# DOGECOIN87/firedancer

Hardware: AMD Instinct MI355X
Metric: verified ed25519 sigs/sec (node) (higher is better)
Workload: dtype u32; 1 GPU; cfg2: 1000000 single-sig txns/GPU, msg U[180,220] B, 90% valid / 10% corrupted, device-resident batch, full verify + per-txn combine per step; parallelism=dp1 (independent per-GPU batches), queues=2

## Files before the change

firedancer_amd/csrc/fdgpu_internal.h:

```cpp
#pragma once

#include <hip/hip_runtime_api.h>
#include <stddef.h>
#include <stdint.h>

#include "../../include/fd_ed25519_gpu.h"
#include "../../include/fd_poh_gpu.h"

typedef struct {
  uint32_t msg_off;
  uint32_t msg_sz;
  uint32_t sig_off;
  uint32_t pub_off;
} fdgpu_sig_desc_t;

typedef struct {
  uint32_t sig0;
  uint32_t sig_cnt;
} fdgpu_txn_desc_t;

#define FDGPU_ARENA_SLACK   160u
#define FDGPU_ATAB_ENTRIES  9u
#ifndef FDGPU_ATAB_WORDS
#define FDGPU_ATAB_WORDS    40u
#endif
#define FDGPU_PTAB_WORDS    32u
#ifndef FDGPU_VERIFY_WAVES
#define FDGPU_VERIFY_WAVES  2
#endif
#ifndef FDGPU_PHASE_STAMPS
#define FDGPU_PHASE_STAMPS  0
#endif
#define FDGPU_BCOMB_BITS    16u
#define FDGPU_BCOMB_NDIG    ((254u + FDGPU_BCOMB_BITS - 1u) / FDGPU_BCOMB_BITS)
#define FDGPU_BCOMB_ENTRIES ((1u << (FDGPU_BCOMB_BITS - 1u)) + 1u)
#define FDGPU_BCOMB_STRIDE  32u
#define FDGPU_BCOMB_CHUNK   64u
#define HS_MAX_WIN          40u
#define FDGPU_TAB_STORED    (FDGPU_ATAB_ENTRIES - 1u)
#define FDGPU_WS_RTAB       FDGPU_TAB_STORED
#define FDGPU_WS_ENTRIES    (2u * FDGPU_TAB_STORED + 2u)
#define FDGPU_WS_LANE_WORDS (FDGPU_WS_ENTRIES * FDGPU_ATAB_WORDS)
#define FDGPU_WS_TAB_WORDS  (2u * FDGPU_TAB_STORED * FDGPU_PTAB_WORDS)
#define FDGPU_WS_AUX_WORDS  (FDGPU_WS_LANE_WORDS - FDGPU_WS_TAB_WORDS)
#define FDGPU_AUX_PARK      0u
#define FDGPU_AUX_SB        FDGPU_ATAB_WORDS
#define FDGPU_BLOCK         256u
#define FDGPU_FLAG_REF_MAP  1u
#define FDGPU_FLAG_KFULL    2u
#define FDGPU_FLAG_KCACHE   4u
#define FDGPU_FLAG_KPAIR    8u
#define FDGPU_FLAG_KSPREAD  16u
#define FDGPU_STAGE_WAVE_WORDS (FDGPU_PTAB_WORDS / 4u * 256u)
#define FDGPU_STAGE_LDS        (FDGPU_BLOCK / 64u * 2u * FDGPU_STAGE_WAVE_WORDS * 4u)
#define FDGPU_STAGE_LDS_PAIR   (FDGPU_BLOCK / 64u * FDGPU_STAGE_WAVE_WORDS * 4u)
#define FDGPU_CU_LDS           (160u * 1024u)
#define FDGPU_SPREAD_LDS       (FDGPU_CU_LDS / 2u - FDGPU_STAGE_LDS + 1024u)
#define FDGPU_SPREAD_LDS_PAIR  (FDGPU_CU_LDS / 2u - FDGPU_STAGE_LDS_PAIR + 1024u)
#ifdef __cplusplus
static_assert(2u * (FDGPU_STAGE_LDS + FDGPU_SPREAD_LDS) > FDGPU_CU_LDS &&
              2u * (FDGPU_STAGE_LDS_PAIR + FDGPU_SPREAD_LDS_PAIR) > FDGPU_CU_LDS &&
              FDGPU_STAGE_LDS + FDGPU_SPREAD_LDS <= FDGPU_CU_LDS && FDGPU_STAGE_LDS_PAIR + FDGPU_SPREAD_LDS_PAIR <= FDGPU_CU_LDS,
              "a spread launch's LDS admits one block per CU, and no more");
#endif
#define FDGPU_FULL_BLOCKS   16u
#define FDGPU_AUX_BLOCKS    64u
#define FDGPU_IO_BLOCKS     16u
#define FDGPU_NBLK_GROUPS   32u
#define FDGPU_POH_CHUNK     64u

#ifdef __cplusplus
extern "C" {
#endif


size_t     fdgpu_btab_bytes(void);
hipError_t fdgpu_btab_build(uint32_t *d_btab, hipStream_t stream);

hipError_t fdgpu_launch_verify_sigs(const uint8_t *d_arena, const fdgpu_sig_desc_t *d_sigs, uint32_t n_sig,
// ... 116 lines not shown
```

firedancer_amd/csrc/fdgpu_verify.hip:

```cpp
#include <hip/hip_runtime.h>

#include "fdgpu_atab.h"
#include "fdgpu_bcomb.h"
#include "fdgpu_ge.h"
#include "fdgpu_hram.h"
#include "fdgpu_internal.h"
#include "fdgpu_lattice.h"
#include "fdgpu_sc.h"
#include "fdgpu_sha512.h"
#include "fdgpu_stamps.h"

using namespace fdgpu;

namespace {


FDG_DEV uint32_t *tab_a(uint32_t *wsl) { return wsl - FDGPU_PTAB_WORDS; }
FDG_DEV const uint32_t *tab_a(const uint32_t *wsl) { return wsl - FDGPU_PTAB_WORDS; }
FDG_DEV uint32_t *tab_r(uint32_t *wsl) { return wsl + (FDGPU_WS_RTAB - 1u) * FDGPU_PTAB_WORDS; }

FDG_DEV void sb_store(uint32_t *aux, const ge_cached &c) {
  uint4 *p = (uint4 *)(aux + FDGPU_AUX_SB);
  uint32_t w[40];
#pragma unroll
  for (int i = 0; i < 10; i++) { w[i] = c.YpX.v[i]; w[10 + i] = c.YmX.v[i]; w[20 + i] = c.Z2.v[i]; w[30 + i] = c.T2d.v[i]; }
#pragma unroll
  for (int q = 0; q < 10; q++) p[q] = make_uint4(w[4 * q], w[4 * q + 1], w[4 * q + 2], w[4 * q + 3]);
}
FDG_DEV void sb_load(uint32_t (&q)[40], const uint32_t *aux) {
  const uint4 *ent = (const uint4 *)(aux + FDGPU_AUX_SB);
#pragma unroll
  for (int i = 0; i < 10; i++) {
    const uint4 v = ent[i];
    q[4 * i] = v.x; q[4 * i + 1] = v.y; q[4 * i + 2] = v.z; q[4 * i + 3] = v.w;
  }
}
FDG_DEV int sext4(uint32_t x) { return ((int)(x << 28)) >> 28; }

#define KD_WORDS 8

FDG_DEV void shl4(uint32_t (&w)[8]) {
#pragma unroll
  for (int i = 7; i > 0; i--) w[i] = (w[i] << 4) | (w[i - 1] >> 28);
  w[0] <<= 4;
}

FDG_DEV void dsm_k(ge_p2 &acc2, uint32_t (&kd)[KD_WORDS], const uint32_t *aux, const uint32_t *ta) {
  ge_p3 acc3;
  ge_p1p1 t;
  uint32_t q[40];
  {
    const int e = sext4(kd[7] >> 28);
    shl4(kd);
    atab_load(q, ta, e);
    ge_cached_regs_to_p2(acc2, q, e < 0);
  }
#pragma unroll 1
  for (int j = 62; j >= 0; j--) {
    const int e = sext4(kd[7] >> 28);
    shl4(kd);
    atab_load(q, ta, e);
#pragma unroll 1
    for (int r = 0; r < 4; r++) {
      ge_dbl(t, acc2);
      ge_p1p1_to_p2(acc2, t);
    }
    acc3.X = acc2.X; acc3.Y = acc2.Y; acc3.Z = acc2.Z; fe_mul(acc3.T, t.X, t.Y);
    ge_add_cached_regs(t, acc3, q, e < 0);
    if (j == 0) break;
    ge_p1p1_to_p2(acc2, t);
  }
  ge_p1p1_to_p3(acc3, t);
  uint32_t qs[40];
  sb_load(qs, aux);
  ge_add_cached_regs(t, acc3, qs, false);
  ge_p1p1_to_p2(acc2, t);
}

FDG_DEV void comb_sb(ge_p3 &acc, const uint32_t (&S)[8], const uint32_t *__restrict__ btab, uint32_t lo = 0,
                     uint32_t hi = BC_NDIG) {
  constexpr int NW = COMB_WORDS(BC_W, BC_NDIG), SLOT = COMB_SLOT(BC_W);
  uint32_t dg[NW];
  sc_recode_comb<(int)BC_W, (int)BC_NDIG>(dg, S);
  auto next_digit = [&dg]() {
    const int d = SLOT == 16 ? (int)(int16_t)(dg[0] & 0xffffu) : (int)dg[0];
#pragma unroll
    for (int i = 0; i < NW - 1; i++) dg[i] = SLOT == 16 ? (dg[i] >> 16) | (dg[i + 1] << 16) : dg[i + 1];
    dg[NW - 1] = SLOT == 16 ? dg[NW - 1] >> 16 : 0u;
    return d;
  };
  auto load_entry = [btab](uint32_t (&q)[32], uint32_t ti, int d) {
    const uint4 *ent = (const uint4 *)(btab + ((size_t)ti * BC_ENT + (uint32_t)(d < 0 ? -d : d)) * FDGPU_BCOMB_STRIDE);
#pragma unroll
    for (int i = 0; i < 8; i++) {
      const uint4 v = ent[i];
      q[4 * i] = v.x; q[4 * i + 1] = v.y; q[4 * i + 2] = v.z; q[4 * i + 3] = v.w;
    }
  };
  uint32_t qa[32], qb[32];
#pragma unroll 1
  for (uint32_t i = 0; i < lo; i++) (void)next_digit();
  int d = next_digit();
  load_entry(qa, lo, d);
  {
    const int dn = next_digit();
    load_entry(qb, lo + 1, dn);
    ge_niels_regs_to_p3(acc, qa, d < 0);
#pragma unroll
    for (int w = 0; w < 32; w++) qa[w] = qb[w];
    d = dn;
  }
  ge_p1p1 t;
#pragma unroll 1
  for (uint32_t i = lo + 1; i < hi; i++) {
    const int dn = next_digit();
    if (i + 1 < hi) load_entry(qb, i + 1, dn);
    ge_add_niels_regs(t, acc, qa, d < 0);
    ge_p1p1_to_p3(acc, t);
#pragma unroll
    for (int w = 0; w < 32; w++) qa[w] = qb[w];
    d = dn;
  }
}

FDG_DEV void atab_build(uint32_t *wsl, const ge_p3 &An) {
  ge_cached c;
  ge_p3_to_cached(c, An); atab_store(wsl, 1, c);
  ge_p1p1 t; ge_p2 a2; ge_p3 P;
  ge_p3_to_p2(a2, An); ge_dbl(t, a2); ge_p1p1_to_p3(P, t);
  ge_p3_to_cached(c, P); atab_store(wsl, 2, c);
  const uint32_t *ent1 = wsl + 1u * FDGPU_PTAB_WORDS;
  auto ld1 = [ent1](int cc, int w) { return atab_limb(ent1, cc, w); };
#pragma unroll 1
  for (uint32_t e = 3; e < FDGPU_ATAB_ENTRIES; e++) {
    if (e & 1u) {
      ge_add_cached_ld(t, P, ld1, false);
    } else {
      uint32_t q[40];
      atab_load(q, wsl, (int)(e >> 1));
      ge_cached_regs_to_p2(a2, q, false);
      ge_dbl(t, a2);
    }
    ge_p1p1_to_p3(P, t);
    ge_p3_to_cached(c, P); atab_store(wsl, e, c);
  }
}

FDG_DEV uint32_t *lane_ws(uint32_t *ws, uint32_t i) {
  return ws + (size_t)i * FDGPU_WS_TAB_WORDS;
}
FDG_DEV uint32_t *lane_aux(uint32_t *queue, uint32_t i) {
  return queue - ((size_t)i + 1u) * FDGPU_WS_AUX_WORDS;
}
FDG_DEV const uint32_t *lane_aux(const uint32_t *queue, uint32_t i) {
  return queue - ((size_t)i + 1u) * FDGPU_WS_AUX_WORDS;
}

FDG_DEV uint32_t out_idx(const uint32_t *__restrict__ perm, uint32_t i) { return perm ? perm[i] : i; }


#define HPARK_KD 0
#define HPARK_CODE 30
static_assert(HPARK_KD + KD_WORDS <= HPARK_CODE && HPARK_CODE < (int)FDGPU_AUX_SB - (int)FDGPU_AUX_PARK &&
              FDGPU_AUX_SB + FDGPU_ATAB_WORDS <= FDGPU_WS_AUX_WORDS && FDGPU_AUX_SB % 4u == 0 && FDGPU_WS_AUX_WORDS % 4u == 0,
              "aux layout");

FDG_DEV void recode16_160(uint32_t (&out)[5], uint32_t &nd, const uint32_t (&m)[5]) {
  uint32_t carry = 0;
  nd = 0;
#pragma unroll
  for (int w = 0; w < 5; w++) {
    uint32_t o = 0;
#pragma unroll
    for (int n = 0; n < 8; n++) {
      uint32_t e = ((m[w] >> (4 * n)) & 15u) + carry;
      carry = e >= 8u;
      e = (e - (carry << 4)) & 15u;
      o |= e << (4 * n);
      nd = e ? (uint32_t)(8 * w + n + 1) : nd;
    }
    out[w] = o;
  }
  nd = carry ? 41u : nd;
}

FDG_DEV void shl4_5(uint32_t (&w)[5]) {
#pragma unroll
  for (int i = 4; i > 0; i--) w[i] = (w[i] << 4) | (w[i - 1] >> 28);
  w[0] <<= 4;
}

FDG_DEV void hs_wscalar(uint32_t (&w)[8], const uint32_t (&v)[5], bool v_neg, const uint32_t (&S)[8]) {
  uint32_t x[16];
#pragma unroll
  for (int i = 0; i < 16; i++) x[i] = 0;
#pragma unroll
  for (int i = 0; i < 5; i++) {
// ... 61 lines not shown
    ge_p1p1_to_p3(acc3, t);
    unstage_entry_signed(q, st_r, (dv < 0) != v_neg);
    ge_add_cached_regs_swapped(t, acc3, q, (dv < 0) != v_neg);
  }
}


FDG_DEV uint32_t decode_neg_table(uint32_t *tab, const uint32_t (&enc)[8], bool ref_map) {
  ge_p3 P, Pn;
  const bool ok = ge_decode(P, enc, ref_map);
  const bool small = ge_is_small_order_affine(P);
  ge_p3_neg(Pn, P);
  atab_build(tab, Pn);
  return (ok ? 1u : 0u) | (small ? 2u : 0u);
}

FDG_DEV void hs_split_masked(hs_split_t &hs, const uint32_t (&k)[8], bool need) {
  uint32_t ke[8];
#pragma unroll
  for (int j = 0; j < 8; j++) ke[j] = need ? k[j] : 0u;
  hs_split(hs, ke);
}

FDG_DEV uint32_t hs_digits(uint32_t (&ud)[5], uint32_t (&vd)[5], const hs_split_t &hs) {
  uint32_t ndu = 0, ndv = 0;
  recode16_160(ud, ndu, hs.u);
  recode16_160(vd, ndv, hs.v);
  return max(max(ndu, ndv), 1u);
}

FDG_DEV void comb_scalar(uint32_t (&w)[8], const hs_split_t &hs, const uint32_t (&S)[8], bool half) {
  hs_wscalar(w, hs.v, hs.v_neg, S);
#pragma unroll
  for (int j = 0; j < 8; j++) w[j] = half ? w[j] : S[j];
}

FDG_DEV void park_full(uint32_t *park, const uint32_t (&k)[8]) {
  uint32_t kd[KD_WORDS];
  sc_recode16(kd, k);
#pragma unroll
  for (int j = 0; j < KD_WORDS; j++) park[HPARK_KD + j] = kd[j];
  park[HPARK_CODE] = 0u;
}

FDG_DEV void queue_full_lanes(uint32_t *queue, uint32_t *queue_cnt, bool q_full, uint32_t i) {
  const uint64_t m = __ballot(q_full);
  if (m) {
    const int lane = (int)(threadIdx.x & 63u);
    const int leader = __ffsll((long long)m) - 1;
    uint32_t base = 0;
    if (lane == leader) base = atomicAdd(queue_cnt, (uint32_t)__popcll(m));
    base = (uint32_t)__shfl((int)base, leader, 64);
    if (q_full) queue[base + (uint32_t)__popcll(m & ((1ull << lane) - 1ull))] = i;
  }
}

template <bool KC, bool PH = false>
FDG_DEV void verify_hs_body(const uint8_t *__restrict__ arena, const fdgpu_sig_desc_t *__restrict__ sigs, uint32_t n_sig_arg,
                            const uint32_t *__restrict__ n_sig_dev, const uint32_t *__restrict__ btab,
                            uint32_t *__restrict__ ws, const uint32_t *__restrict__ perm, int8_t *__restrict__ codes,
                            uint32_t *__restrict__ queue, uint32_t *__restrict__ queue_cnt, uint32_t flags,
                            const uint32_t *__restrict__ key_of, const uint32_t *__restrict__ kverd, uint32_t bx) {
  const uint32_t n_sig = n_sig_dev ? *n_sig_dev : n_sig_arg;
  if (bx * blockDim.x >= n_sig) return;
  const uint32_t i = bx * blockDim.x + threadIdx.x;
  const bool active = i < n_sig;
  const bool ref_map = (flags & FDGPU_FLAG_REF_MAP) != 0;
  const fdgpu_sig_desc_t d = sigs[active ? i : n_sig - 1];
  uint32_t nb = sha512_hram_blocks(d.msg_sz);
#pragma unroll
  for (int off = 32; off > 0; off >>= 1) nb = max(nb, (uint32_t)__shfl_xor((int)nb, off));
  uint32_t *wsl = lane_ws(ws, i);
  uint32_t *aux = lane_aux(queue, i);
  const uint32_t *ta = tab_a(wsl);
  FDGPU_STAMP(0);
  uint32_t Renc[8], Aenc[8];
  load32(Renc, arena + d.sig_off);
  load32(Aenc, arena + d.pub_off);
  uint32_t k[8];
  {
    uint64_t h[8];
    if (PH) {
#pragma unroll
      for (int j = 0; j < 8; j++) h[j] = ((const uint64_t *)(arena + d.msg_off))[j];
    } else {
      sha512_hram(h, Renc, Aenc, arena + d.msg_off, d.msg_sz, nb);
    }
    FDGPU_STAMP(1);
    uint32_t kx[16];
#pragma unroll
    for (int j = 0; j < 8; j++) { kx[2 * j] = bswap32((uint32_t)(h[j] >> 32)); kx[2 * j + 1] = bswap32((uint32_t)h[j]); }
    sc_reduce512(k, kx);
  }
  uint32_t S[8];
  load32(S, arena + d.sig_off + 32);
  int code = sc_lt_L(S) ? 0 : -1;
#pragma unroll
  for (int j = 0; j < 8; j++) S[j] = code ? 0u : S[j];
  FDGPU_STAMP(2);
  {
    ge_p3 P, Pn;
    bool a_ok, a_small;
    if (KC) {
      const uint32_t di = active ? i : n_sig - 1u, r = key_of[di], vd = kverd[r];
      a_ok = (vd & 1u) != 0;
      a_small = (vd & 2u) != 0;
      ta = tab_a(lane_ws(ws, r));
    } else {
      a_ok = ge_decode(P, Aenc, ref_map);
      a_small = ge_is_small_order_affine(P);
      ge_p3_neg(Pn, P);
      atab_build(tab_a(wsl), Pn);
    }
    FDGPU_STAMP(3);
    const bool r_ok = ge_decode(P, Renc, ref_map);
    const bool r_small = ge_is_small_order_affine(P);
    ge_p3_neg(Pn, P);
    atab_build(tab_r(wsl), Pn);
    if (code == 0 && !a_ok) code = ref_map ? -2 : -1;
    if (code == 0 && !r_ok) code = -1;
    if (code == 0 && a_small) code = -2;
    if (code == 0 && r_small) code = -1;
  }
  FDGPU_STAMP(4);
  const bool need = active && code == 0;
  hs_split_t hs;
  hs_split_masked(hs, k, need);
  uint32_t ud[5], vd[5];
  const uint32_t nd_lane = hs_digits(ud, vd, hs);
  const bool full = need && (!hs.ok || nd_lane > HS_MAX_WIN || (flags & FDGPU_FLAG_KFULL));
  const bool half = need && !full;
  FDGPU_STAMP(5);
  {
    uint32_t w[8];
    comb_scalar(w, hs, S, half);
    ge_p3 WB;
    comb_sb(WB, w, btab);
    ge_cached c; ge_p3_to_cached(c, WB);
    sb_store(aux, c);
  }
  if (full) park_full(aux + FDGPU_AUX_PARK, k);
  FDGPU_STAMP(6);
  bool eq = false;
  if (__any(half)) {
    const uint32_t nwin = wave_max_u32(half ? nd_lane : 1u);
#pragma unroll 1
    for (uint32_t s = nwin; s < 40; s++) { shl4_5(ud); shl4_5(vd); }
    ge_p1p1 t;
    hs_chain(t, ud, vd, hs.u_neg, hs.v_neg, nwin, wsl, ta);
    uint32_t q[40];
    sb_load(q, aux);
    fe ypx, ymx, z2, xw, yw, l1, l2;
#pragma unroll
    for (int j = 0; j < 10; j++) { ypx.v[j] = q[j]; ymx.v[j] = q[10 + j]; z2.v[j] = q[20 + j]; }
    fe_sub(xw, ypx, ymx);
    fe_add(yw, ypx, ymx);
    fe_mul(l1, t.X, z2);
    fe_mul(l2, t.Z, xw);
    fe_add(l1, l1, l2);
    const bool ex = fe_iszero(l1);
    fe_mul(l1, t.Y, z2);
    fe_mul(l2, t.T, yw);
    fe_sub(l1, l1, l2);
    eq = ex && fe_iszero(l1);
  }
  FDGPU_STAMP(7);
  if (active && !full) codes[out_idx(perm, i)] = (int8_t)(code ? code : (eq ? 0 : -3));
  queue_full_lanes(queue, queue_cnt, full, i);
}

template <bool KC, bool PH = false>
__global__ void __launch_bounds__(FDGPU_BLOCK, FDGPU_VERIFY_WAVES)
fdgpu_verify_hs_kernel(const uint8_t *__restrict__ arena, const fdgpu_sig_desc_t *__restrict__ sigs, uint32_t n_sig_arg,
                       const uint32_t *__restrict__ n_sig_dev, const uint32_t *__restrict__ btab,
                       uint32_t *__restrict__ ws, const uint32_t *__restrict__ perm, int8_t *__restrict__ codes,
                       uint32_t *__restrict__ queue, uint32_t *__restrict__ queue_cnt, uint32_t flags,
                       const uint32_t *__restrict__ key_of, const uint32_t *__restrict__ kverd) {
  verify_hs_body<KC, PH>(arena, sigs, n_sig_arg, n_sig_dev, btab, ws, perm, codes, queue, queue_cnt, flags, key_of,
                         kverd, blockIdx.x);
}

__global__ void __launch_bounds__(64) fdgpu_sha512_stream_kernel(const uint8_t *__restrict__ mbuf, uint64_t m0,
                                                                 uint64_t mlen, uint64_t msg_sz, uint64_t blk0,
                                                                 uint32_t nblk, const uint8_t *__restrict__ ra,
                                                                 uint64_t *__restrict__ state, uint32_t n) {
  const uint32_t i = threadIdx.x;
  if (i >= n) return;
  const uint64_t H0[8] = {0x6a09e667f3bcc908ULL, 0xbb67ae8584caa73bULL, 0x3c6ef372fe94f82bULL,
                          0xa54ff53a5f1d36f1ULL, 0x510e527fade682d1ULL, 0x9b05688c2b3e6c1fULL,
                          0x1f83d9abfb41bd6bULL, 0x5be0cd19137e2179ULL};
  uint64_t h[8];
  for (int j = 0; j < 8; j++) h[j] = blk0 ? state[8 * i + j] : H0[j];
  const uint64_t total = (64u + msg_sz + 16u) / 128u + 1u, bitlen = (64u + msg_sz) * 8u;
  for (uint64_t b = blk0; b < blk0 + nblk; b++) {
    uint64_t w[16];
    for (int t = 0; t < 16; t++) {
      uint64_t v = 0;
// ... 47 lines not shown
    stage_entry(st, tab, d);
#pragma unroll 1
    for (int r = 0; r < 4; r++) {
      ge_dbl(t, acc2);
      ge_p1p1_to_p2(acc2, t);
    }
    acc3.X = acc2.X; acc3.Y = acc2.Y; acc3.Z = acc2.Z; fe_mul(acc3.T, t.X, t.Y);
    asm volatile("s_waitcnt vmcnt(0)" ::: "memory");
    unstage_entry_signed(q, st, (d < 0) != neg);
    ge_add_cached_regs_swapped(t, acc3, q, (d < 0) != neg);
  }
}

FDG_DEV void fe_xchg_pair(fe &r, const fe &a) {
#pragma unroll
  for (int j = 0; j < 10; j++) r.v[j] = (uint32_t)__shfl_xor((int)a.v[j], 1);
}

template <bool PH = false>
__global__ void __launch_bounds__(FDGPU_BLOCK, FDGPU_VERIFY_WAVES)
fdgpu_verify_pair_kernel(const uint8_t *__restrict__ arena, const fdgpu_sig_desc_t *__restrict__ sigs, uint32_t n_sig_arg,
                         const uint32_t *__restrict__ n_sig_dev, const uint32_t *__restrict__ btab,
                         uint32_t *__restrict__ ws, const uint32_t *__restrict__ perm, int8_t *__restrict__ codes,
                         uint32_t *__restrict__ queue, uint32_t *__restrict__ queue_cnt, uint32_t flags) {
  const uint32_t n_sig = n_sig_dev ? *n_sig_dev : n_sig_arg;
  if (blockIdx.x * (blockDim.x / 2u) >= n_sig) return;
  const uint32_t g = blockIdx.x * blockDim.x + threadIdx.x, i = g >> 1;
  const bool rl = (g & 1u) != 0;
  const bool active = i < n_sig;
  const bool ref_map = (flags & FDGPU_FLAG_REF_MAP) != 0;
  const fdgpu_sig_desc_t d = sigs[active ? i : n_sig - 1];
  const uint32_t nb = wave_max_u32(sha512_hram_blocks(d.msg_sz));
  uint32_t *wsl = lane_ws(ws, i);
  uint32_t *aux = lane_aux(queue, i);
  uint32_t *tab = rl ? tab_r(wsl) : tab_a(wsl);
  uint32_t Renc[8], Aenc[8];
  load32(Renc, arena + d.sig_off);
  load32(Aenc, arena + d.pub_off);
  uint32_t k[8];
  if (PH) {
    uint32_t kx[16];
#pragma unroll
    for (int j = 0; j < 8; j++) {
      const uint64_t h = ((const uint64_t *)(arena + d.msg_off))[j];
      kx[2 * j] = bswap32((uint32_t)(h >> 32)); kx[2 * j + 1] = bswap32((uint32_t)h);
    }
    sc_reduce512(k, kx);
  } else {
    hram_k(k, Renc, Aenc, arena, d, nb);
  }
  uint32_t S[8];
  load32(S, arena + d.sig_off + 32);
  int code = sc_lt_L(S) ? 0 : -1;
#pragma unroll
  for (int j = 0; j < 8; j++) S[j] = code ? 0u : S[j];
  {
    uint32_t enc[8];
#pragma unroll
    for (int j = 0; j < 8; j++) enc[j] = rl ? Renc[j] : Aenc[j];
    const uint32_t mine = decode_neg_table(tab, enc, ref_map);
    const uint32_t other = (uint32_t)__shfl_xor((int)mine, 1);
    const uint32_t av = rl ? other : mine, rv = rl ? mine : other;
    if (code == 0 && !(av & 1u)) code = ref_map ? -2 : -1;
    if (code == 0 && !(rv & 1u)) code = -1;
    if (code == 0 && (av & 2u)) code = -2;
    if (code == 0 && (rv & 2u)) code = -1;
  }
  const bool need = active && code == 0;
  hs_split_t hs;
  hs_split_masked(hs, k, need);
  uint32_t ud[5], vd[5];
  const uint32_t nd_lane = hs_digits(ud, vd, hs);
  const bool full = need && (!hs.ok || nd_lane > HS_MAX_WIN || (flags & FDGPU_FLAG_KFULL));
  const bool half = need && !full;
  {
    uint32_t w[8];
    comb_scalar(w, hs, S, half);
    ge_p3 WB, WBo;
    comb_sb(WB, w, btab, rl ? BC_NDIG / 2u : 0u, rl ? BC_NDIG : BC_NDIG / 2u);
    fe_xchg_pair(WBo.X, WB.X);
    fe_xchg_pair(WBo.Y, WB.Y);
    fe_xchg_pair(WBo.Z, WB.Z);
    fe_xchg_pair(WBo.T, WB.T);
    ge_cached c; ge_p3_to_cached(c, WBo);
    ge_p1p1 tw; ge_add_cached(tw, WB, c, false);
    ge_p1p1_to_p3(WB, tw);
    ge_p3_to_cached(c, WB);
    if (!rl) sb_store(aux, c);
  }
  if (full && !rl) park_full(aux + FDGPU_AUX_PARK, k);
  bool eq = false;
  if (__any(half)) {
    const uint32_t nwin = wave_max_u32(half ? nd_lane : 1u);
    uint32_t dd[5];
#pragma unroll
    for (int j = 0; j < 5; j++) dd[j] = rl ? vd[j] : ud[j];
#pragma unroll 1
    for (uint32_t s2 = nwin; s2 < 40; s2++) shl4_5(dd);
    ge_p1p1 t;
    hs_chain1(t, dd, rl ? hs.v_neg : hs.u_neg, nwin, tab);
    ge_p3 mine, other;
    ge_p1p1_to_p3(mine, t);
    fe_xchg_pair(other.X, mine.X);
    fe_xchg_pair(other.Y, mine.Y);
    fe_xchg_pair(other.Z, mine.Z);
    fe_xchg_pair(other.T, mine.T);
    ge_cached oc;
    ge_p3_to_cached(oc, other);
    ge_add_cached(t, mine, oc, false);
    uint32_t q[40];
    sb_load(q, aux);
    fe ypx, ymx, z2, xw, yw, l1, l2;
#pragma unroll
    for (int j = 0; j < 10; j++) { ypx.v[j] = q[j]; ymx.v[j] = q[10 + j]; z2.v[j] = q[20 + j]; }
    fe_sub(xw, ypx, ymx);
    fe_add(yw, ypx, ymx);
    fe_mul(l1, t.X, z2);
    fe_mul(l2, t.Z, xw);
    fe_add(l1, l1, l2);
    const bool ex = fe_iszero(l1);
    fe_mul(l1, t.Y, z2);
    fe_mul(l2, t.T, yw);
    fe_sub(l1, l1, l2);
    eq = ex && fe_iszero(l1);
  }
  if (active && !full && !rl) codes[out_idx(perm, i)] = (int8_t)(code ? code : (eq ? 0 : -3));
  queue_full_lanes(queue, queue_cnt, full && !rl, i);
}

#define KC_PROBES 32u
#define KC_EMPTY 0xffffffffu

FDG_DEV uint32_t kc_hash(const uint32_t (&a)[8], uint64_t seed) {
  uint64_t h = seed;
#pragma unroll
  for (int j = 0; j < 4; j++) {
    h ^= ((uint64_t)a[2 * j + 1] << 32) | a[2 * j];
    h *= 0x9e3779b97f4a7c15ull;
    h ^= h >> 29;
  }
  h *= 0xbf58476d1ce4e5b9ull;
  return (uint32_t)(h >> 32) ^ (uint32_t)h;
}

__global__ void __launch_bounds__(256) fdgpu_key_dedup_kernel(const uint8_t *__restrict__ arena,
                                                              const fdgpu_sig_desc_t *__restrict__ sigs,
                                                              uint32_t n_sig_arg, const uint32_t *__restrict__ n_sig_dev,
                                                              uint32_t *__restrict__ ht, uint32_t ht_mask,
                                                              uint32_t *__restrict__ key_of, uint32_t *__restrict__ reps,
                                                              uint32_t *__restrict__ rep_cnt, uint64_t seed) {
  const uint32_t n_sig = n_sig_dev ? *n_sig_dev : n_sig_arg;
  if (blockIdx.x * blockDim.x >= n_sig) return;
  const uint32_t i = blockIdx.x * blockDim.x + threadIdx.x;
  bool is_rep = false;
  if (i < n_sig) {
    uint32_t a[8];
    load32(a, arena + sigs[i].pub_off);
// ... 10 lines not shown
#pragma unroll
      for (int j = 0; j < 8; j++) diff |= a[j] ^ b[j];
      if (!diff) { rep = v; break; }
    }
    key_of[i] = rep;
    is_rep = rep == i;
  }
  __shared__ uint32_t s_cnt, s_base;
  if (threadIdx.x == 0) s_cnt = 0;
  __syncthreads();
  const uint64_t m = __ballot(is_rep);
  const int lane = (int)(threadIdx.x & 63u);
  uint32_t wbase = 0;
  if (m && lane == __ffsll((long long)m) - 1) wbase = atomicAdd(&s_cnt, (uint32_t)__popcll(m));
  if (m) wbase = (uint32_t)__shfl((int)wbase, __ffsll((long long)m) - 1, 64);
  __syncthreads();
  if (threadIdx.x == 0) s_base = s_cnt ? atomicAdd(rep_cnt, s_cnt) : 0u;
  __syncthreads();
  if (is_rep) reps[s_base + wbase + (uint32_t)__popcll(m & ((1ull << lane) - 1ull))] = i;
}

__global__ void __launch_bounds__(FDGPU_BLOCK, FDGPU_VERIFY_WAVES)
fdgpu_key_table_kernel(const uint8_t *__restrict__ arena, const fdgpu_sig_desc_t *__restrict__ sigs,
                       uint32_t *__restrict__ ws, const uint32_t *__restrict__ reps,
                       const uint32_t *__restrict__ rep_cnt, uint32_t *__restrict__ kverd, uint32_t flags) {
  const uint32_t q = blockIdx.x * blockDim.x + threadIdx.x;
  if (q >= *rep_cnt) return;
  const uint32_t i = reps[q];
  uint32_t Aenc[8];
  load32(Aenc, arena + sigs[i].pub_off);
  kverd[i] = decode_neg_table(tab_a(lane_ws(ws, i)), Aenc, (flags & FDGPU_FLAG_REF_MAP) != 0);
}

__global__ void __launch_bounds__(FDGPU_BLOCK, FDGPU_VERIFY_WAVES)
fdgpu_full_kernel(uint32_t *__restrict__ ws, const uint32_t *__restrict__ perm, int8_t *__restrict__ codes,
                  const uint32_t *__restrict__ queue, const uint32_t *__restrict__ queue_cnt, uint32_t slots,
                  const uint32_t *__restrict__ key_of);

FDG_DEV void full_body(uint32_t *__restrict__ ws, const uint32_t *__restrict__ perm, int8_t *__restrict__ codes,
                       const uint32_t *__restrict__ queue, const uint32_t *__restrict__ queue_cnt, uint32_t slots,
                       const uint32_t *__restrict__ key_of, uint32_t bx) {
  const uint32_t cnt = *queue_cnt;
  if (bx * blockDim.x >= cnt) return;
  for (uint32_t q = bx * blockDim.x + threadIdx.x; q < cnt; q += slots) {
    const uint32_t i = queue[q];
    uint32_t *wsl = lane_ws(ws, i);
    const uint32_t *aux = lane_aux(queue, i), *park = aux + FDGPU_AUX_PARK;
    uint32_t kd[KD_WORDS];
#pragma unroll
    for (int j = 0; j < KD_WORDS; j++) kd[j] = park[HPARK_KD + j];
    ge_p2 Rc;
    dsm_k(Rc, kd, aux, tab_a(key_of ? lane_ws(ws, key_of[i]) : wsl));
    uint32_t er[40];
    atab_load(er, tab_r(wsl), 1);
    fe ypx, ymx, z2, x2, y2, l, r;
#pragma unroll
    for (int j = 0; j < 10; j++) { ypx.v[j] = er[j]; ymx.v[j] = er[10 + j]; z2.v[j] = er[20 + j]; }
    fe_carry(ypx); fe_carry(ymx); fe_carry(z2);
    fe_sub(x2, ymx, ypx);
    fe_add(y2, ypx, ymx);
    fe_mul(l, Rc.X, z2); fe_mul(r, x2, Rc.Z);
    bool eq = fe_eq(l, r);
    fe_mul(l, Rc.Y, z2); fe_mul(r, y2, Rc.Z);
    eq = eq && fe_eq(l, r);
    codes[out_idx(perm, i)] = (int8_t)(eq ? 0 : -3);
  }
}

__global__ void __launch_bounds__(FDGPU_BLOCK, FDGPU_VERIFY_WAVES)
fdgpu_full_kernel(uint32_t *__restrict__ ws, const uint32_t *__restrict__ perm, int8_t *__restrict__ codes,
                  const uint32_t *__restrict__ queue, const uint32_t *__restrict__ queue_cnt, uint32_t slots,
                  const uint32_t *__restrict__ key_of) {
  full_body(ws, perm, codes, queue, queue_cnt, slots, key_of, blockIdx.x);
}

__global__ void __launch_bounds__(FDGPU_BLOCK, FDGPU_VERIFY_WAVES)
fdgpu_full_multi_kernel(const fdgpu_mbatch_t *__restrict__ mb) {
  const fdgpu_mbatch_t b = mb[blockIdx.y];
  if (blockIdx.x >= b.slow) return;
  full_body(b.ws, nullptr, b.codes, b.queue, b.cnt, b.slow * FDGPU_BLOCK, nullptr, blockIdx.x);
}

__global__ void __launch_bounds__(256) fdgpu_combine_kernel(const fdgpu_txn_desc_t *__restrict__ txns, uint32_t n_txn,
                                                            const int8_t *__restrict__ sig_codes,
                                                            int8_t *__restrict__ txn_codes,
                                                            uint64_t *__restrict__ accept) {
  for (uint32_t t0 = blockIdx.x * blockDim.x; t0 < n_txn; t0 += gridDim.x * blockDim.x) {
    const uint32_t t = t0 + threadIdx.x;
    int code = -1;
    if (t < n_txn) {
      const fdgpu_txn_desc_t d = txns[t];
      if (d.sig_cnt >= 1 && d.sig_cnt <= 16) {
        int first_struct = 0, any_msg = 0;
        for (uint32_t j = 0; j < d.sig_cnt; j++) {
          const int c = sig_codes[d.sig0 + j];
          if (c == -3) any_msg = 1;
          else if (c != 0 && first_struct == 0) first_struct = c;
        }
        code = first_struct ? first_struct : (any_msg ? -3 : 0);
      }
      txn_codes[t] = (int8_t)code;
    }
    const uint64_t ok = __ballot(t < n_txn && code == 0);
    if (accept && (threadIdx.x & 63u) == 0 && t < n_txn) accept[t >> 6] = ok;
  }
}

}

extern "C" {

char const *fdgpu_kernel_path(void) { return "halfsize: fdgpu_verify_hs_kernel + fdgpu_full_kernel"; }

// ... 14 lines not shown
                                    int8_t *d_sig_codes, uint32_t flags, hipStream_t stream, const uint32_t *d_n_sig,
                                    uint32_t resident_blocks, uint64_t kc_seed, int cnt_zeroed) {
  if (!n_sig) return hipSuccess;
  const uint32_t grid = (n_sig + FDGPU_BLOCK - 1) / FDGPU_BLOCK;
  const fdgpu_ws_layout_t l = fdgpu_ws_layout(d_ws, n_sig);
  hipError_t e = cnt_zeroed ? hipSuccess : hipMemsetAsync(l.cnt, 0, sizeof(uint32_t), stream);
  if (e != hipSuccess) return e;
  if (!resident_blocks) resident_blocks = 1;
  uint32_t slow_blocks = grid < resident_blocks ? grid : resident_blocks;
  const uint32_t slow_cap = grid > 64u ? FDGPU_FULL_BLOCKS : FDGPU_FULL_BLOCKS / 4u;
  if (slow_blocks > slow_cap) slow_blocks = slow_cap;
  const uint32_t *key_of = nullptr;
  if (flags & FDGPU_FLAG_KCACHE) {
    e = hipMemsetAsync(l.ht, 0xff, l.ht_slots * sizeof(uint32_t), stream);
    if (e == hipSuccess) e = hipMemsetAsync(l.rep_cnt, 0, sizeof(uint32_t), stream);
    if (e != hipSuccess) return e;
    hipLaunchKernelGGL(fdgpu_key_dedup_kernel, dim3((n_sig + 255) / 256), dim3(256), 0, stream, d_arena, d_sigs, n_sig,
                       d_n_sig, l.ht, (uint32_t)(l.ht_slots - 1), l.key_of, l.reps, l.rep_cnt, kc_seed);
    hipLaunchKernelGGL(fdgpu_key_table_kernel, dim3(grid), dim3(FDGPU_BLOCK), 0, stream, d_arena, d_sigs, d_ws, l.reps,
                       l.rep_cnt, l.kverd, flags);
    hipLaunchKernelGGL(fdgpu_verify_hs_kernel<true>, dim3(grid), dim3(FDGPU_BLOCK), 0, stream, d_arena, d_sigs, n_sig,
                       d_n_sig, d_btab, d_ws, d_perm, d_sig_codes, l.queue, l.cnt, flags, l.key_of, l.kverd);
    key_of = l.key_of;
  } else if (flags & FDGPU_FLAG_KPAIR) {
    const uint32_t pgrid = (2u * n_sig + FDGPU_BLOCK - 1) / FDGPU_BLOCK;
    hipLaunchKernelGGL(fdgpu_verify_pair_kernel<false>, dim3(pgrid), dim3(FDGPU_BLOCK),
                       (flags & FDGPU_FLAG_KSPREAD) ? FDGPU_SPREAD_LDS_PAIR : 0, stream, d_arena, d_sigs, n_sig,
                       d_n_sig, d_btab, d_ws, d_perm, d_sig_codes, l.queue, l.cnt, flags);
  } else {
    hipLaunchKernelGGL(fdgpu_verify_hs_kernel<false>, dim3(grid), dim3(FDGPU_BLOCK),
                       (flags & FDGPU_FLAG_KSPREAD) ? FDGPU_SPREAD_LDS : 0, stream, d_arena, d_sigs, n_sig,
                       d_n_sig, d_btab, d_ws, d_perm, d_sig_codes, l.queue, l.cnt, flags, nullptr, nullptr);
  }
  hipLaunchKernelGGL(fdgpu_full_kernel, dim3(slow_blocks), dim3(FDGPU_BLOCK), 0, stream, d_ws, d_perm, d_sig_codes,
                     l.queue, l.cnt, slow_blocks * FDGPU_BLOCK, key_of);
  return hipGetLastError();
}

uint64_t fdgpu_sha512_stream_blocks(uint64_t msg_sz) { return (64u + msg_sz + 16u) / 128u + 1u; }

hipError_t fdgpu_launch_sha512_stream(const uint8_t *d_mbuf, uint64_t m0, uint64_t mlen, uint64_t msg_sz,
                                      uint64_t blk0, uint32_t nblk, const uint8_t *d_ra, uint64_t *d_state,
                                      uint32_t n, hipStream_t stream) {
  if (!n || n > 64 || !nblk) return hipErrorInvalidValue;
  hipLaunchKernelGGL(fdgpu_sha512_stream_kernel, dim3(1), dim3(64), 0, stream, d_mbuf, m0, mlen, msg_sz, blk0, nblk,
                     d_ra, d_state, n);
  return hipGetLastError();
}

hipError_t fdgpu_launch_verify_prehashed(const uint8_t *d_arena, const fdgpu_sig_desc_t *d_sigs, uint32_t n_sig,
                                         const uint32_t *d_btab, uint32_t *d_ws, int8_t *d_sig_codes, uint32_t flags,
                                         hipStream_t stream) {
  if (!n_sig) return hipSuccess;
  const uint32_t grid = (n_sig + FDGPU_BLOCK - 1) / FDGPU_BLOCK;
  const fdgpu_ws_layout_t l = fdgpu_ws_layout(d_ws, n_sig);
  hipError_t e = hipMemsetAsync(l.cnt, 0, sizeof(uint32_t), stream);
  if (e != hipSuccess) return e;
  const uint32_t kf = flags & (FDGPU_FLAG_REF_MAP | FDGPU_FLAG_KFULL);
  if (flags & FDGPU_FLAG_KPAIR) {
    const uint32_t pgrid = (2u * n_sig + FDGPU_BLOCK - 1) / FDGPU_BLOCK;
    hipLaunchKernelGGL(fdgpu_verify_pair_kernel<true>, dim3(pgrid), dim3(FDGPU_BLOCK), 0, stream, d_arena, d_sigs,
                       n_sig, nullptr, d_btab, d_ws, nullptr, d_sig_codes, l.queue, l.cnt, kf);
  } else {
    hipLaunchKernelGGL((fdgpu_verify_hs_kernel<false, true>), dim3(grid), dim3(FDGPU_BLOCK), 0, stream, d_arena, d_sigs,
                       n_sig, nullptr, d_btab, d_ws, nullptr, d_sig_codes, l.queue, l.cnt, kf, nullptr, nullptr);
  }
  hipLaunchKernelGGL(fdgpu_full_kernel, dim3(1), dim3(FDGPU_BLOCK), 0, stream, d_ws, nullptr, d_sig_codes, l.queue,
                     l.cnt, FDGPU_BLOCK, nullptr);
  return hipGetLastError();
}

hipError_t fdgpu_launch_verify_multi(const fdgpu_mbatch_t *mb, uint32_t nb, uint32_t grid_max, uint32_t slow_max,
                                     const uint32_t *d_btab, uint32_t flags, hipStream_t stream) {
  if (!nb || !grid_max) return hipSuccess;
  hipLaunchKernelGGL(fdgpu_verify_hs_multi_kernel, dim3(grid_max, nb), dim3(FDGPU_BLOCK), 0, stream, mb, d_btab, flags);
  hipLaunchKernelGGL(fdgpu_full_multi_kernel, dim3(slow_max ? slow_max : 1, nb), dim3(FDGPU_BLOCK), 0, stream, mb);
  return hipGetLastError();
}

hipError_t fdgpu_launch_combine(const fdgpu_txn_desc_t *d_txns, uint32_t n_txn, const int8_t *d_sig_codes,
                                int8_t *d_txn_codes, uint64_t *d_accept, hipStream_t stream) {
  if (!n_txn) return hipSuccess;
  const uint32_t blocks = (n_txn + 255) / 256;
  hipLaunchKernelGGL(fdgpu_combine_kernel, dim3(blocks < FDGPU_AUX_BLOCKS ? blocks : FDGPU_AUX_BLOCKS), dim3(256), 0,
                     stream, d_txns, n_txn, d_sig_codes, d_txn_codes, d_accept);
  return hipGetLastError();
}

#if FDGPU_PHASE_STAMPS
int fdgpu_debug_stamps(uint64_t *out, uint64_t n_waves) {
  if (n_waves > FDGPU_STAMP_WAVES) n_waves = FDGPU_STAMP_WAVES;
  return hipMemcpyFromSymbol(out, HIP_SYMBOL(g_fdgpu_stamps), n_waves * FDGPU_STAMP_SLOTS * sizeof(uint64_t)) ==
                 hipSuccess ? 0 : -1;
}
#endif

}
```

Before: 109.3 million sigs/s.

## Accumulate fixed-base comb directly onto chain result instead of storing separate point

The fixed-base comb multiplication is no longer computed into a separate point, converted to cached form and stored in per-lane aux memory. Instead it starts from the half-size chain result and adds the comb entries onto it, and the final check becomes an identity test. Full-path lanes park S and recompute the comb inside the slow kernel. This removes one point conversion, the global store and reload of the cached point, and the projective equality check. In exchange the full kernel now does the comb work and needs the btab table, and the comb adds now sit in the dependent chain after hs_chain.

New measurement: 110.0 million sigs/s (median of 6 runs). Within noise of the previous version (+0.6%).

```diff
diff --git a/firedancer_amd/csrc/fdgpu_internal.h b/firedancer_amd/csrc/fdgpu_internal.h
--- a/firedancer_amd/csrc/fdgpu_internal.h
+++ b/firedancer_amd/csrc/fdgpu_internal.h
@@ -44,7 +44,7 @@
 #define FDGPU_WS_TAB_WORDS  (2u * FDGPU_TAB_STORED * FDGPU_PTAB_WORDS)
 #define FDGPU_WS_AUX_WORDS  (FDGPU_WS_LANE_WORDS - FDGPU_WS_TAB_WORDS)
 #define FDGPU_AUX_PARK      0u
-#define FDGPU_AUX_SB        FDGPU_ATAB_WORDS
+#define FDGPU_AUX_PARK_WORDS FDGPU_ATAB_WORDS
 #define FDGPU_BLOCK         256u
 #define FDGPU_FLAG_REF_MAP  1u
 #define FDGPU_FLAG_KFULL    2u
diff --git a/firedancer_amd/csrc/fdgpu_verify.hip b/firedancer_amd/csrc/fdgpu_verify.hip
--- a/firedancer_amd/csrc/fdgpu_verify.hip
+++ b/firedancer_amd/csrc/fdgpu_verify.hip
@@ -19,22 +19,6 @@
 FDG_DEV const uint32_t *tab_a(const uint32_t *wsl) { return wsl - FDGPU_PTAB_WORDS; }
 FDG_DEV uint32_t *tab_r(uint32_t *wsl) { return wsl + (FDGPU_WS_RTAB - 1u) * FDGPU_PTAB_WORDS; }
 
-FDG_DEV void sb_store(uint32_t *aux, const ge_cached &c) {
-  uint4 *p = (uint4 *)(aux + FDGPU_AUX_SB);
-  uint32_t w[40];
-#pragma unroll
-  for (int i = 0; i < 10; i++) { w[i] = c.YpX.v[i]; w[10 + i] = c.YmX.v[i]; w[20 + i] = c.Z2.v[i]; w[30 + i] = c.T2d.v[i]; }
-#pragma unroll
-  for (int q = 0; q < 10; q++) p[q] = make_uint4(w[4 * q], w[4 * q + 1], w[4 * q + 2], w[4 * q + 3]);
-}
-FDG_DEV void sb_load(uint32_t (&q)[40], const uint32_t *aux) {
-  const uint4 *ent = (const uint4 *)(aux + FDGPU_AUX_SB);
-#pragma unroll
-  for (int i = 0; i < 10; i++) {
-    const uint4 v = ent[i];
-    q[4 * i] = v.x; q[4 * i + 1] = v.y; q[4 * i + 2] = v.z; q[4 * i + 3] = v.w;
-  }
-}
 FDG_DEV int sext4(uint32_t x) { return ((int)(x << 28)) >> 28; }
 
 #define KD_WORDS 8
@@ -45,7 +29,52 @@
   w[0] <<= 4;
 }
 
-FDG_DEV void dsm_k(ge_p2 &acc2, uint32_t (&kd)[KD_WORDS], const uint32_t *aux, const uint32_t *ta) {
+FDG_DEV void comb_sb_onto(ge_p1p1 &t, ge_p3 &acc, const uint32_t (&S)[8], const uint32_t *__restrict__ btab,
+                          uint32_t lo = 0, uint32_t hi = BC_NDIG) {
+  constexpr int NW = COMB_WORDS(BC_W, BC_NDIG), SLOT = COMB_SLOT(BC_W);
+  uint32_t dg[NW];
+  sc_recode_comb<(int)BC_W, (int)BC_NDIG>(dg, S);
+  auto next_digit = [&dg]() {
+    const int d = SLOT == 16 ? (int)(int16_t)(dg[0] & 0xffffu) : (int)dg[0];
+#pragma unroll
+    for (int i = 0; i < NW - 1; i++) dg[i] = SLOT == 16 ? (dg[i] >> 16) | (dg[i + 1] << 16) : dg[i + 1];
+    dg[NW - 1] = SLOT == 16 ? dg[NW - 1] >> 16 : 0u;
+    return d;
+  };
+  auto load_entry = [btab](uint32_t (&q)[32], uint32_t ti, int d) {
+    const uint4 *ent = (const uint4 *)(btab + ((size_t)ti * BC_ENT + (uint32_t)(d < 0 ? -d : d)) * FDGPU_BCOMB_STRIDE);
+#pragma unroll
+    for (int i = 0; i < 8; i++) {
+      const uint4 v = ent[i];
+      q[4 * i] = v.x; q[4 * i + 1] = v.y; q[4 * i + 2] = v.z; q[4 * i + 3] = v.w;
+    }
+  };
+  uint32_t qa[32], qb[32];
+#pragma unroll 1
+  for (uint32_t i = 0; i < lo; i++) (void)next_digit();
+  int d = next_digit();
+  load_entry(qa, lo, d);
+#pragma unroll 1
+  for (uint32_t i = lo;; i++) {
+    const int dn = next_digit();
+    if (i + 1 < hi) load_entry(qb, i + 1, dn);
+    ge_add_niels_regs(t, acc, qa, d < 0);
+    if (i + 1 >= hi) break;
+    ge_p1p1_to_p3(acc, t);
+#pragma unroll
+    for (int w = 0; w < 32; w++) qa[w] = qb[w];
+    d = dn;
+  }
+}
+
+FDG_DEV bool ge_p1p1_is_identity(const ge_p1p1 &t) {
+  fe hf;
+  fe_sub(hf, t.Y, t.T);
+  return fe_iszero(t.X) && fe_iszero(hf);
+}
+
+FDG_DEV void dsm_k(ge_p2 &acc2, uint32_t (&kd)[KD_WORDS], const uint32_t (&S)[8], const uint32_t *ta,
+                   const uint32_t *__restrict__ btab) {
   ge_p3 acc3;
   ge_p1p1 t;
   uint32_t q[40];
@@ -71,56 +100,8 @@
     ge_p1p1_to_p2(acc2, t);
   }
   ge_p1p1_to_p3(acc3, t);
-  uint32_t qs[40];
-  sb_load(qs, aux);
-  ge_add_cached_regs(t, acc3, qs, false);
+  comb_sb_onto(t, acc3, S, btab);
   ge_p1p1_to_p2(acc2, t);
-}
-
-FDG_DEV void comb_sb(ge_p3 &acc, const uint32_t (&S)[8], const uint32_t *__restrict__ btab, uint32_t lo = 0,
-                     uint32_t hi = BC_NDIG) {
-  constexpr int NW = COMB_WORDS(BC_W, BC_NDIG), SLOT = COMB_SLOT(BC_W);
-  uint32_t dg[NW];
-  sc_recode_comb<(int)BC_W, (int)BC_NDIG>(dg, S);
-  auto next_digit = [&dg]() {
-    const int d = SLOT == 16 ? (int)(int16_t)(dg[0] & 0xffffu) : (int)dg[0];
-#pragma unroll
-    for (int i = 0; i < NW - 1; i++) dg[i] = SLOT == 16 ? (dg[i] >> 16) | (dg[i + 1] << 16) : dg[i + 1];
-    dg[NW - 1] = SLOT == 16 ? dg[NW - 1] >> 16 : 0u;
-    return d;
-  };
-  auto load_entry = [btab](uint32_t (&q)[32], uint32_t ti, int d) {
-    const uint4 *ent = (const uint4 *)(btab + ((size_t)ti * BC_ENT + (uint32_t)(d < 0 ? -d : d)) * FDGPU_BCOMB_STRIDE);
-#pragma unroll
-    for (int i = 0; i < 8; i++) {
-      const uint4 v = ent[i];
-      q[4 * i] = v.x; q[4 * i + 1] = v.y; q[4 * i + 2] = v.z; q[4 * i + 3] = v.w;
-    }
-  };
-  uint32_t qa[32], qb[32];
-#pragma unroll 1
-  for (uint32_t i = 0; i < lo; i++) (void)next_digit();
-  int d = next_digit();
-  load_entry(qa, lo, d);
-  {
-    const int dn = next_digit();
-    load_entry(qb, lo + 1, dn);
-    ge_niels_regs_to_p3(acc, qa, d < 0);
-#pragma unroll
-    for (int w = 0; w < 32; w++) qa[w] = qb[w];
-    d = dn;
-  }
-  ge_p1p1 t;
-#pragma unroll 1
-  for (uint32_t i = lo + 1; i < hi; i++) {
-    const int dn = next_digit();
-    if (i + 1 < hi) load_entry(qb, i + 1, dn);
-    ge_add_niels_regs(t, acc, qa, d < 0);
-    ge_p1p1_to_p3(acc, t);
-#pragma unroll
-    for (int w = 0; w < 32; w++) qa[w] = qb[w];
-    d = dn;
-  }
 }
 
 FDG_DEV void atab_build(uint32_t *wsl, const ge_p3 &An) {
@@ -160,9 +141,10 @@
 
 
 #define HPARK_KD 0
+#define HPARK_S 8
 #define HPARK_CODE 30
-static_assert(HPARK_KD + KD_WORDS <= HPARK_CODE && HPARK_CODE < (int)FDGPU_AUX_SB - (int)FDGPU_AUX_PARK &&
-              FDGPU_AUX_SB + FDGPU_ATAB_WORDS <= FDGPU_WS_AUX_WORDS && FDGPU_AUX_SB % 4u == 0 && FDGPU_WS_AUX_WORDS % 4u == 0,
+static_assert(HPARK_KD + KD_WORDS <= HPARK_S && HPARK_S + 8 <= HPARK_CODE && HPARK_CODE < (int)FDGPU_AUX_PARK_WORDS &&
+              FDGPU_AUX_PARK + FDGPU_AUX_PARK_WORDS <= FDGPU_WS_AUX_WORDS,
               "aux layout");
 
 FDG_DEV void recode16_160(uint32_t (&out)[5], uint32_t &nd, const uint32_t (&m)[5]) {
@@ -290,14 +272,16 @@
 FDG_DEV void comb_scalar(uint32_t (&w)[8], const hs_split_t &hs, const uint32_t (&S)[8], bool half) {
   hs_wscalar(w, hs.v, hs.v_neg, S);
 #pragma unroll
-  for (int j = 0; j < 8; j++) w[j] = half ? w[j] : S[j];
-}
-
-FDG_DEV void park_full(uint32_t *park, const uint32_t (&k)[8]) {
+  for (int j = 0; j < 8; j++) w[j] = half ? w[j] : 0u;
+}
+
+FDG_DEV void park_full(uint32_t *park, const uint32_t (&k)[8], const uint32_t (&S)[8]) {
   uint32_t kd[KD_WORDS];
   sc_recode16(kd, k);
 #pragma unroll
   for (int j = 0; j < KD_WORDS; j++) park[HPARK_KD + j] = kd[j];
+#pragma unroll
+  for (int j = 0; j < 8; j++) park[HPARK_S + j] = S[j];
   park[HPARK_CODE] = 0u;
 }
 
@@ -329,7 +313,6 @@
 #pragma unroll
   for (int off = 32; off > 0; off >>= 1) nb = max(nb, (uint32_t)__shfl_xor((int)nb, off));
   uint32_t *wsl = lane_ws(ws, i);
-  uint32_t *aux = lane_aux(queue, i);
   const uint32_t *ta = tab_a(wsl);
   FDGPU_STAMP(0);
   uint32_t Renc[8], Aenc[8];
@@ -389,15 +372,9 @@
   const bool full = need && (!hs.ok || nd_lane > HS_MAX_WIN || (flags & FDGPU_FLAG_KFULL));
   const bool half = need && !full;
   FDGPU_STAMP(5);
-  {
-    uint32_t w[8];
-    comb_scalar(w, hs, S, half);
-    ge_p3 WB;
-    comb_sb(WB, w, btab);
-    ge_cached c; ge_p3_to_cached(c, WB);
-    sb_store(aux, c);
-  }
-  if (full) park_full(aux + FDGPU_AUX_PARK, k);
+  uint32_t w[8];
+  comb_scalar(w, hs, S, half);
+  if (full) park_full(lane_aux(queue, i) + FDGPU_AUX_PARK, k, S);
   FDGPU_STAMP(6);
   bool eq = false;
   if (__any(half)) {
@@ -406,21 +383,10 @@
     for (uint32_t s = nwin; s < 40; s++) { shl4_5(ud); shl4_5(vd); }
     ge_p1p1 t;
     hs_chain(t, ud, vd, hs.u_neg, hs.v_neg, nwin, wsl, ta);
-    uint32_t q[40];
-    sb_load(q, aux);
-    fe ypx, ymx, z2, xw, yw, l1, l2;
-#pragma unroll
-    for (int j = 0; j < 10; j++) { ypx.v[j] = q[j]; ymx.v[j] = q[10 + j]; z2.v[j] = q[20 + j]; }
-    fe_sub(xw, ypx, ymx);
-    fe_add(yw, ypx, ymx);
-    fe_mul(l1, t.X, z2);
-    fe_mul(l2, t.Z, xw);
-    fe_add(l1, l1, l2);
-    const bool ex = fe_iszero(l1);
-    fe_mul(l1, t.Y, z2);
-    fe_mul(l2, t.T, yw);
-    fe_sub(l1, l1, l2);
-    eq = ex && fe_iszero(l1);
+    ge_p3 C;
+    ge_p1p1_to_p3(C, t);
+    comb_sb_onto(t, C, w, btab);
+    eq = ge_p1p1_is_identity(t);
   }
   FDGPU_STAMP(7);
   if (active && !full) codes[out_idx(perm, i)] = (int8_t)(code ? code : (eq ? 0 : -3));
@@ -534,7 +500,6 @@
   const fdgpu_sig_desc_t d = sigs[active ? i : n_sig - 1];
   const uint32_t nb = wave_max_u32(sha512_hram_blocks(d.msg_sz));
   uint32_t *wsl = lane_ws(ws, i);
-  uint32_t *aux = lane_aux(queue, i);
   uint32_t *tab = rl ? tab_r(wsl) : tab_a(wsl);
   uint32_t Renc[8], Aenc[8];
   load32(Renc, arena + d.sig_off);
@@ -575,22 +540,9 @@
   const uint32_t nd_lane = hs_digits(ud, vd, hs);
   const bool full = need && (!hs.ok || nd_lane > HS_MAX_WIN || (flags & FDGPU_FLAG_KFULL));
   const bool half = need && !full;
-  {
-    uint32_t w[8];
-    comb_scalar(w, hs, S, half);
-    ge_p3 WB, WBo;
-    comb_sb(WB, w, btab, rl ? BC_NDIG / 2u : 0u, rl ? BC_NDIG : BC_NDIG / 2u);
-    fe_xchg_pair(WBo.X, WB.X);
-    fe_xchg_pair(WBo.Y, WB.Y);
-    fe_xchg_pair(WBo.Z, WB.Z);
-    fe_xchg_pair(WBo.T, WB.T);
-    ge_cached c; ge_p3_to_cached(c, WBo);
-    ge_p1p1 tw; ge_add_cached(tw, WB, c, false);
-    ge_p1p1_to_p3(WB, tw);
-    ge_p3_to_cached(c, WB);
-    if (!rl) sb_store(aux, c);
-  }
-  if (full && !rl) park_full(aux + FDGPU_AUX_PARK, k);
+  uint32_t w[8];
+  comb_scalar(w, hs, S, half);
+  if (full && !rl) park_full(lane_aux(queue, i) + FDGPU_AUX_PARK, k, S);
   bool eq = false;
   if (__any(half)) {
     const uint32_t nwin = wave_max_u32(half ? nd_lane : 1u);
@@ -602,6 +554,8 @@
     ge_p1p1 t;
     hs_chain1(t, dd, rl ? hs.v_neg : hs.u_neg, nwin, tab);
     ge_p3 mine, other;
+    ge_p1p1_to_p3(mine, t);
+    comb_sb_onto(t, mine, w, btab, rl ? BC_NDIG / 2u : 0u, rl ? BC_NDIG : BC_NDIG / 2u);
     ge_p1p1_to_p3(mine, t);
     fe_xchg_pair(other.X, mine.X);
     fe_xchg_pair(other.Y, mine.Y);
@@ -610,21 +564,8 @@
     ge_cached oc;
     ge_p3_to_cached(oc, other);
     ge_add_cached(t, mine, oc, false);
-    uint32_t q[40];
-    sb_load(q, aux);
-    fe ypx, ymx, z2, xw, yw, l1, l2;
-#pragma unroll
-    for (int j = 0; j < 10; j++) { ypx.v[j] = q[j]; ymx.v[j] = q[10 + j]; z2.v[j] = q[20 + j]; }
-    fe_sub(xw, ypx, ymx);
-    fe_add(yw, ypx, ymx);
-    fe_mul(l1, t.X, z2);
-    fe_mul(l2, t.Z, xw);
-    fe_add(l1, l1, l2);
-    const bool ex = fe_iszero(l1);
-    fe_mul(l1, t.Y, z2);
-    fe_mul(l2, t.T, yw);
-    fe_sub(l1, l1, l2);
-    eq = ex && fe_iszero(l1);
+    fe_carry(t.T);
+    eq = ge_p1p1_is_identity(t);
   }
   if (active && !full && !rl) codes[out_idx(perm, i)] = (int8_t)(code ? code : (eq ? 0 : -3));
   queue_full_lanes(queue, queue_cnt, full && !rl, i);
@@ -701,25 +642,23 @@
   kverd[i] = decode_neg_table(tab_a(lane_ws(ws, i)), Aenc, (flags & FDGPU_FLAG_REF_MAP) != 0);
 }
 
-__global__ void __launch_bounds__(FDGPU_BLOCK, FDGPU_VERIFY_WAVES)
-fdgpu_full_kernel(uint32_t *__restrict__ ws, const uint32_t *__restrict__ perm, int8_t *__restrict__ codes,
-                  const uint32_t *__restrict__ queue, const uint32_t *__restrict__ queue_cnt, uint32_t slots,
-                  const uint32_t *__restrict__ key_of);
-
-FDG_DEV void full_body(uint32_t *__restrict__ ws, const uint32_t *__restrict__ perm, int8_t *__restrict__ codes,
-                       const uint32_t *__restrict__ queue, const uint32_t *__restrict__ queue_cnt, uint32_t slots,
-                       const uint32_t *__restrict__ key_of, uint32_t bx) {
+FDG_DEV void full_body(uint32_t *__restrict__ ws, const uint32_t *__restrict__ btab, const uint32_t *__restrict__ perm,
+                       int8_t *__restrict__ codes, const uint32_t *__restrict__ queue,
+                       const uint32_t *__restrict__ queue_cnt, uint32_t slots, const uint32_t *__restrict__ key_of,
+                       uint32_t bx) {
   const uint32_t cnt = *queue_cnt;
   if (bx * blockDim.x >= cnt) return;
   for (uint32_t q = bx * blockDim.x + threadIdx.x; q < cnt; q += slots) {
     const uint32_t i = queue[q];
     uint32_t *wsl = lane_ws(ws, i);
-    const uint32_t *aux = lane_aux(queue, i), *park = aux + FDGPU_AUX_PARK;
-    uint32_t kd[KD_WORDS];
+    const uint32_t *park = lane_aux(queue, i) + FDGPU_AUX_PARK;
+    uint32_t kd[KD_WORDS], S[8];
 #pragma unroll
     for (int j = 0; j < KD_WORDS; j++) kd[j] = park[HPARK_KD + j];
+#pragma unroll
+    for (int j = 0; j < 8; j++) S[j] = park[HPARK_S + j];
     ge_p2 Rc;
-    dsm_k(Rc, kd, aux, tab_a(key_of ? lane_ws(ws, key_of[i]) : wsl));
+    dsm_k(Rc, kd, S, tab_a(key_of ? lane_ws(ws, key_of[i]) : wsl), btab);
     uint32_t er[40];
     atab_load(er, tab_r(wsl), 1);
     fe ypx, ymx, z2, x2, y2, l, r;
@@ -737,17 +676,17 @@
 }
 
 __global__ void __launch_bounds__(FDGPU_BLOCK, FDGPU_VERIFY_WAVES)
-fdgpu_full_kernel(uint32_t *__restrict__ ws, const uint32_t *__restrict__ perm, int8_t *__restrict__ codes,
-                  const uint32_t *__restrict__ queue, const uint32_t *__restrict__ queue_cnt, uint32_t slots,
-                  const uint32_t *__restrict__ key_of) {
-  full_body(ws, perm, codes, queue, queue_cnt, slots, key_of, blockIdx.x);
+fdgpu_full_kernel(uint32_t *__restrict__ ws, const uint32_t *__restrict__ btab, const uint32_t *__restrict__ perm,
+                  int8_t *__restrict__ codes, const uint32_t *__restrict__ queue,
+                  const uint32_t *__restrict__ queue_cnt, uint32_t slots, const uint32_t *__restrict__ key_of) {
+  full_body(ws, btab, perm, codes, queue, queue_cnt, slots, key_of, blockIdx.x);
 }
 
 __global__ void __launch_bounds__(FDGPU_BLOCK, FDGPU_VERIFY_WAVES)
-fdgpu_full_multi_kernel(const fdgpu_mbatch_t *__restrict__ mb) {
+fdgpu_full_multi_kernel(const fdgpu_mbatch_t *__restrict__ mb, const uint32_t *__restrict__ btab) {
   const fdgpu_mbatch_t b = mb[blockIdx.y];
   if (blockIdx.x >= b.slow) return;
-  full_body(b.ws, nullptr, b.codes, b.queue, b.cnt, b.slow * FDGPU_BLOCK, nullptr, blockIdx.x);
+  full_body(b.ws, btab, nullptr, b.codes, b.queue, b.cnt, b.slow * FDGPU_BLOCK, nullptr, blockIdx.x);
 }
 
 __global__ void __launch_bounds__(256) fdgpu_combine_kernel(const fdgpu_txn_desc_t *__restrict__ txns, uint32_t n_txn,
@@ -828,8 +767,8 @@
                        (flags & FDGPU_FLAG_KSPREAD) ? FDGPU_SPREAD_LDS : 0, stream, d_arena, d_sigs, n_sig,
                        d_n_sig, d_btab, d_ws, d_perm, d_sig_codes, l.queue, l.cnt, flags, nullptr, nullptr);
   }
-  hipLaunchKernelGGL(fdgpu_full_kernel, dim3(slow_blocks), dim3(FDGPU_BLOCK), 0, stream, d_ws, d_perm, d_sig_codes,
-                     l.queue, l.cnt, slow_blocks * FDGPU_BLOCK, key_of);
+  hipLaunchKernelGGL(fdgpu_full_kernel, dim3(slow_blocks), dim3(FDGPU_BLOCK), 0, stream, d_ws, d_btab, d_perm,
+                     d_sig_codes, l.queue, l.cnt, slow_blocks * FDGPU_BLOCK, key_of);
   return hipGetLastError();
 }
 
@@ -861,8 +800,8 @@
     hipLaunchKernelGGL((fdgpu_verify_hs_kernel<false, true>), dim3(grid), dim3(FDGPU_BLOCK), 0, stream, d_arena, d_sigs,
                        n_sig, nullptr, d_btab, d_ws, nullptr, d_sig_codes, l.queue, l.cnt, kf, nullptr, nullptr);
   }
-  hipLaunchKernelGGL(fdgpu_full_kernel, dim3(1), dim3(FDGPU_BLOCK), 0, stream, d_ws, nullptr, d_sig_codes, l.queue,
-                     l.cnt, FDGPU_BLOCK, nullptr);
+  hipLaunchKernelGGL(fdgpu_full_kernel, dim3(1), dim3(FDGPU_BLOCK), 0, stream, d_ws, d_btab, nullptr, d_sig_codes,
+                     l.queue, l.cnt, FDGPU_BLOCK, nullptr);
   return hipGetLastError();
 }
 
@@ -870,7 +809,8 @@
                                      const uint32_t *d_btab, uint32_t flags, hipStream_t stream) {
   if (!nb || !grid_max) return hipSuccess;
   hipLaunchKernelGGL(fdgpu_verify_hs_multi_kernel, dim3(grid_max, nb), dim3(FDGPU_BLOCK), 0, stream, mb, d_btab, flags);
-  hipLaunchKernelGGL(fdgpu_full_multi_kernel, dim3(slow_max ? slow_max : 1, nb), dim3(FDGPU_BLOCK), 0, stream, mb);
+  hipLaunchKernelGGL(fdgpu_full_multi_kernel, dim3(slow_max ? slow_max : 1, nb), dim3(FDGPU_BLOCK), 0, stream, mb,
+                     d_btab);
   return hipGetLastError();
 }
 
```
